# VITA-Group/NeRF-SOS

Hardware: AMD Instinct MI355X
Metric: rays/sec (coarse+fine, 64+128 samples) (higher is better)
Workload: dtype f32; 1 GPU; BASELINE configs[1]: LLFF flower_full shape, 4096 rays/GPU x (64 coarse + 192 fine MLP evaluations), eval-mode NeRFNet.forward, fp32 exact-MFMA, no semantic head, random-init weights (seed 0), pinhole rays 1008x756 f=850; rays_per_gpu=4096, parallelism=ray-sharded x1, no collective in the path

## Files before the change

nerf-sos_amd/csrc/lp_common.h:

```cpp
#pragma once
#include "mlp_common.h"
#include "mlp_host.h"

namespace nsos {
namespace lp {

typedef unsigned u32x4 __attribute__((ext_vector_type(4)));
typedef unsigned u32x2 __attribute__((ext_vector_type(2)));
typedef _Float16 f16x8 __attribute__((ext_vector_type(8)));
typedef __bf16 bf16x8 __attribute__((ext_vector_type(8)));


constexpr int kSlotGroups = 36;
constexpr int kSlotBytes = kSlotGroups * 1024;
constexpr int kSlots = 4;
constexpr int kDmaPieces = kSlotGroups / 4;
constexpr int kTilePts = 256;
#ifdef NSOS_LP_RING
constexpr int kRing = NSOS_LP_RING, kPre = NSOS_LP_RING + 3, kMid = 2;
#else
constexpr int kRing = 5, kPre = 8, kMid = 2;
#endif

constexpr int kAuxAlphaW = 0;
// ... 18 lines not shown
        return __builtin_amdgcn_mfma_f32_32x32x16_f16(__builtin_bit_cast(f16x8, a), __builtin_bit_cast(f16x8, b), c, 0, 0, 0);
    }
    __device__ static __forceinline__ f32x4 mfma_k32(u32x4 a, u32x4 b, f32x4 c) {
        return __builtin_amdgcn_mfma_f32_16x16x32_f16(__builtin_bit_cast(f16x8, a), __builtin_bit_cast(f16x8, b), c, 0, 0, 0);
    }
    __device__ static __forceinline__ unsigned pack2(float lo, float hi) {
        unsigned r;
        asm volatile("v_cvt_pk_f16_f32 %0, %1, %2" : "=v"(r) : "v"(lo), "v"(hi));
        return r;
    }
    __device__ static __forceinline__ float dot2(unsigned a, unsigned b, float acc) {
        asm volatile("v_dot2c_f32_f16 %0, %1, %2" : "+v"(acc) : "v"(a), "v"(b));
        return acc;
    }
    __device__ static __forceinline__ unsigned short bits(float x) {
        const _Float16 h = (_Float16)x;
        return __builtin_bit_cast(unsigned short, h);
    }
};
struct BF16 {
    static constexpr bool kIsF16 = false;
    __device__ static __forceinline__ float lo(unsigned w) { return __builtin_bit_cast(float, w << 16); }
    __device__ static __forceinline__ float hi(unsigned w) { return __builtin_bit_cast(float, w & 0xffff0000u); }
    static constexpr unsigned kOnes = 0x3F803F80u;
    __device__ static __forceinline__ f32x16 mfma(u32x4 a, u32x4 b, f32x16 c) {
        return __builtin_amdgcn_mfma_f32_32x32x16_bf16(__builtin_bit_cast(bf16x8, a), __builtin_bit_cast(bf16x8, b), c, 0, 0, 0);
    }
    __device__ static __forceinline__ f32x4 mfma_k32(u32x4 a, u32x4 b, f32x4 c) {
        return __builtin_amdgcn_mfma_f32_16x16x32_bf16(__builtin_bit_cast(bf16x8, a), __builtin_bit_cast(bf16x8, b), c, 0, 0, 0);
    }
    __device__ static __forceinline__ unsigned pack2(float lo, float hi) {
        unsigned r;
        asm volatile("v_cvt_pk_bf16_f32 %0, %1, %2" : "=v"(r) : "v"(lo), "v"(hi));
        return r;
    }
    __device__ static __forceinline__ float dot2(unsigned a, unsigned b, float acc) {
        asm volatile("v_dot2c_f32_bf16 %0, %1, %2" : "+v"(acc) : "v"(a), "v"(b));
        return acc;
    }
    __device__ static __forceinline__ unsigned short bits(float x) {
        unsigned u = __builtin_bit_cast(unsigned, x);
        if ((u & 0x7fffffffu) > 0x7f800000u) return (unsigned short)((u >> 16) | 0x40);
        u += 0x7fffu + ((u >> 16) & 1u);
        return (unsigned short)(u >> 16);
    }
};

#define NSOS_LP_QUAD(CVT, RELU_OPS)                                                                                  \
    asm volatile("v_accvgpr_read_b32 %0, %8\n\tv_accvgpr_read_b32 %4, %9\n\t"                                        \
                 "v_accvgpr_read_b32 %1, %10\n\tv_accvgpr_read_b32 %5, %11\n\t"                                      \
                 "v_accvgpr_read_b32 %2, %12\n\tv_accvgpr_read_b32 %6, %13\n\t"                                      \
                 "v_accvgpr_read_b32 %3, %14\n\tv_accvgpr_read_b32 %7, %15\n\t" CVT " %0, %0, %4\n\t" CVT          \
                 " %1, %1, %5\n\t" CVT " %2, %2, %6\n\t" CVT " %3, %3, %7" RELU_OPS                                 \
                 : "=&v"(r0), "=&v"(r1), "=&v"(r2), "=&v"(r3), "=&v"(t0), "=&v"(t1), "=&v"(t2), "=&v"(t3)            \
                 : "a"(z[0]), "a"(z[1]), "a"(z[2]), "a"(z[3]), "a"(z[4]), "a"(z[5]), "a"(z[6]), "a"(z[7]))
#define NSOS_LP_RELU4 "\n\tv_pk_max_i16 %0, %0, 0\n\tv_pk_max_i16 %1, %1, 0\n\tv_pk_max_i16 %2, %2, 0\n\tv_pk_max_i16 %3, %3, 0"
template <class T, bool RELU>
__device__ __forceinline__ u32x4 pack8_acc(const float (&z)[8]) {
    unsigned r0, r1, r2, r3, t0, t1, t2, t3;
    if constexpr (T::kIsF16) {
        if constexpr (RELU) NSOS_LP_QUAD("v_cvt_pk_f16_f32", NSOS_LP_RELU4); else NSOS_LP_QUAD("v_cvt_pk_f16_f32", "");
    } else {
        if constexpr (RELU) NSOS_LP_QUAD("v_cvt_pk_bf16_f32", NSOS_LP_RELU4); else NSOS_LP_QUAD("v_cvt_pk_bf16_f32", "");
    }
    return u32x4{r0, r1, r2, r3};
}

struct LpParams {
    const unsigned* aux;
    const unsigned char* chunks;
    const float* rays_o;
    const float* rays_d;
    const float* viewdirs;
    const float* z_vals;
    float* raw;
    long long n_pts;
    int n_samples;
    int n_tiles;
    unsigned long long* prof;
    float* sem_in;
    unsigned* sem_in16;
    float* sem_hid;
    unsigned* sem_hid16;
};
constexpr int kProfSlots = 64;

struct SliceHalf {
    __host__ __device__ static constexpr int of(int idx) { return (idx >> 3) & 1; }
};

template <class T, int L, int S, bool ONE_AT_63>
__device__ __forceinline__ u32x4 enc_slice(const Enc<L, SliceHalf>& e, const float (&x)[3], int kg) {
    u32x4 out;
    static_for<0, 4>([&](auto qc) {
        constexpr int q = decltype(qc)::value, f0 = 16 * S + 2 * q, f1 = 16 * S + 8 + 2 * q;
        const float lo_a = e.template feature<f0, 0>(x), lo_b = e.template feature<f0 + 1, 0>(x);
        const float hi_a = e.template feature<f1, 1>(x);
        const float hi_b = (ONE_AT_63 && f1 + 1 == 63) ? 1.0f : e.template feature<f1 + 1, 1>(x);
        out[q] = T::pack2(kg ? hi_a : lo_a, kg ? hi_b : lo_b);
    });
    return out;
}


template <class T, int NT, bool RELU>
__device__ __forceinline__ void activate(u32x4 (&H)[2][2 * NT], const f32x16 (&Z)[2][NT]) {
    asm volatile("s_nop 15\n\ts_nop 3" ::: "memory");
#pragma unroll
    for (int c = 0; c < 2; ++c)
#pragma unroll
        for (int t = 0; t < NT; ++t)
#pragma unroll
            for (int u = 0; u < 2; ++u) {
                float z[8];
#pragma unroll
                for (int i = 0; i < 8; ++i) z[i] = Z[c][t][8 * u + i];
                H[c][2 * t + u] = pack8_acc<T, RELU>(z);
            }
}

template <int NT, int NO>
__device__ __forceinline__ void heads_partial_f32(const f32x16 (&h)[NT], const float* w_lane, float (&part)[NO]) {
    asm volatile("s_nop 15\n\ts_nop 3" ::: "memory");
#pragma unroll
    for (int t = 0; t < NT; ++t)
#pragma unroll
        for (int q = 0; q < 4; ++q) {
            f32x4 w[NO];
#pragma unroll
            for (int o = 0; o < NO; ++o) w[o] = *reinterpret_cast<const f32x4*>(w_lane + o * 128 + t * 16 + q * 4);
#pragma unroll
            for (int j = 0; j < 4; ++j) {
                float x;
                asm volatile("v_accvgpr_read_b32 %0, %1\n\tv_max_f32 %0, 0, %0" : "=v"(x) : "a"(h[t][q * 4 + j]));
#pragma unroll
                for (int o = 0; o < NO; ++o) part[o] = __fmaf_rn(w[o][j], x, part[o]);
            }
        }
}

template <class F>
int32_t dispatch_lp(int32_t sem_mode, int32_t dtype, bool save, F&& f) {
    return nsos_dispatch_sem(sem_mode, [&](auto sem) -> int32_t {
        return nsos_dispatch_dtype<F16, BF16>(dtype, [&](auto t) -> int32_t {
            return nsos_dispatch_bool(save, [&](auto sv) -> int32_t {
                if constexpr (decltype(sem)::value == 0 && decltype(sv)::value != 0) return NSOS_ERR_UNSUPPORTED;
                else return f(t, sem, sv);
            });
        });
    });
}

__host__ __device__ constexpr int lp16_chunks(int sem) {
    return 1 + 28 + 5 + (sem ? 3 : 1) + 2;
}
constexpr int kLp16TailBytes = 4096;
__host__ __device__ constexpr size_t lp16_stream_bytes(int sem) { return (size_t)lp16_chunks(sem) * kSlotBytes + kLp16TailBytes; }
int32_t launch_lp16(const LpParams& p, int32_t sem_mode, int32_t dtype, bool save, hipStream_t stream);
int32_t pack_lp16(const void* tensors, int32_t sem_mode, bool is_f16, unsigned char* chunks, hipStream_t stream, bool heads_only = false);

}
}
```

nerf-sos_amd/csrc/mlp_lp16.hip:

```cpp
#include "lp_common.h"
#include "lp16_sched.h"

using namespace nsos;
using namespace nsos::lp;

namespace {

constexpr int kRgbLds = kSlots * kSlotBytes + kAuxWords * 4 + kW16 * 768;
template <class T, int NS, int L, int ONE_AT>
__device__ __forceinline__ void encode16(u32x4 (&out)[NS], const float (&x)[3], const unsigned char* lds_tab, int q) {
    constexpr float kInvHi = 0.15915493667125702f, kInvLo = 6.4206382679e-9f;
    float uh[3], ul[3];
#pragma unroll
    for (int c = 0; c < 3; ++c) {
        uh[c] = x[c] * kInvHi;
        ul[c] = __fmaf_rn(x[c], kInvHi, -uh[c]) + x[c] * kInvLo;
    }
    const float amax = fmaxf(fmaxf(fabsf(x[0]), fabsf(x[1])), fabsf(x[2])) * (float)(1 << (L - 1));
    const bool big = !(amax < 32768.0f);
    float val[8 * NS];
    const f32x4* tab = reinterpret_cast<const f32x4*>(lds_tab) + q * (8 * NS);
    static_for<0, 8 * NS>([&](auto jc) {
        constexpr int j = decltype(jc)::value;
        const f32x4 t = tab[j];
        const float ah = __fmaf_rn(uh[2], t[2], __fmaf_rn(uh[1], t[1], uh[0] * t[0]));
        const float fr = __builtin_amdgcn_fractf(ah);
        const float g = __fmaf_rn(ul[0], t[0], __fmaf_rn(ul[1], t[1], __fmaf_rn(ul[2], t[2], fr))) + t[3];
        val[j] = __builtin_amdgcn_sinf(g);
    });
    if (__builtin_expect(big, 0)) {
        static_for<0, 8 * NS>([&](auto jc) {
            constexpr int j = decltype(jc)::value;
            const f32x4 t = tab[j];
            const float a = __fmaf_rn(x[2], t[2], __fmaf_rn(x[1], t[1], x[0] * t[0]));
            float sn, cs;
            sincosf(a, &sn, &cs);
            val[j] = t[3] != 0.0f ? cs : sn;
        });
    }
#pragma unroll
    for (int e = 0; e < 3; ++e) val[e] = q == 0 ? x[e] : val[e];
    constexpr int one_slot = 8 * (NS - 1) + (ONE_AT - 32 * (NS - 1) - 24);
    static_assert(one_slot >= 8 * (NS - 1) && one_slot < 8 * NS, "the constant input lives in lane group 3 of the last slice");
    val[one_slot] = q == 3 ? 1.0f : val[one_slot];
#pragma unroll
    for (int s = 0; s < NS; ++s)
#pragma unroll
        for (int w = 0; w < 4; ++w) out[s][w] = T::pack2(val[8 * s + 2 * w], val[8 * s + 2 * w + 1]);
}

template <class T, int SEM, bool SAVE = false, bool PROF = false>
__global__ __launch_bounds__(64 * kW16, 1) void mlp_lp16_kernel(const LpParams P) {
    extern __shared__ __attribute__((aligned(16))) unsigned char lds[];
    const int lane0 = threadIdx.x & 63, wave = threadIdx.x >> 6;
    constexpr int NCH = lp16_chunks(SEM);
    constexpr int C = SEM ? 6 : 4;

    const unsigned lds_base = (unsigned)(size_t)(__attribute__((address_space(3))) unsigned char*)lds;
    const int wave_s = __builtin_amdgcn_readfirstlane(wave);
    const unsigned voff = (unsigned)(lane0 * 16);
    auto lane_addr = [&](int b) { return lds_base + (unsigned)(b * kSlotBytes + lane0 * 16); };
    auto slot_addr = [&](int b) { return lds_base + (unsigned)(b * kSlotBytes); };
    unsigned c0 = lane_addr(0), c1 = lane_addr(1), c2 = lane_addr(2), c3 = lane_addr(3);
    unsigned d0 = slot_addr(0), d1 = slot_addr(1), d2 = slot_addr(2), d3 = slot_addr(3);
    const unsigned woff = (unsigned)wave_s * 1024u;
    const unsigned wlast = wave_s + kW16 * kFull16 < kSlotGroups ? woff + (unsigned)(kW16 * kFull16) * 1024u : (unsigned)(kSlotGroups - 1) * 1024u;
    auto poff = [&](int i) { return i < kFull16 ? woff + (unsigned)(kW16 * 1024) * (unsigned)i : wlast; };
    const unsigned char* const src_end = P.chunks + (size_t)NCH * kSlotBytes;
    const unsigned char* srcf = P.chunks + (size_t)(2 % NCH) * kSlotBytes;
    auto dma_piece = [&](const unsigned char* src_chunk, unsigned dst_slot, int i) {
        const unsigned long long sp = (unsigned long long)(src_chunk + poff(i));
        const unsigned lo = __builtin_amdgcn_readfirstlane((unsigned)sp), hi = __builtin_amdgcn_readfirstlane((unsigned)(sp >> 32));
        const unsigned dst = __builtin_amdgcn_readfirstlane(dst_slot + poff(i));
        dma_1k(reinterpret_cast<const void*>(((unsigned long long)hi << 32) | lo), dst, voff);
    };
#ifdef NSOS_LP16_DMA_STAGGER
    unsigned fill_wlast = 0;
#endif
    unsigned fill_lo = 0, fill_hi = 0, fill_dst = 0, fill_w = 0;
#ifdef NSOS_LP16_DMA_STAGGER
    auto side = [&](auto early_c, auto late_c) {
        constexpr int EARLY = decltype(early_c)::value, LATE = decltype(late_c)::value;
        auto piece = [&](int i) {
            const unsigned off = i < kFull16 ? fill_w + (unsigned)(kW16 * 1024) * (unsigned)i : fill_wlast;
            const unsigned long long sp = (((unsigned long long)fill_hi << 32) | fill_lo) + off;
            dma_1k(reinterpret_cast<const void*>(sp), fill_dst + off, voff);
        };
        if constexpr (EARLY >= 0 && EARLY < kDma16) { if (wave_s < 4) { NSOS_PIN(); piece(EARLY); NSOS_PIN(); } }
        if constexpr (LATE >= 0 && LATE < kDma16) { if (wave_s >= 4) { NSOS_PIN(); piece(LATE); NSOS_PIN(); } }
    };
#else
    auto side = [&](int i, int nfill) {
        const unsigned off = fill_w + (unsigned)(kW16 * 1024) * (unsigned)i;
        const unsigned long long sp = (((unsigned long long)fill_hi << 32) | fill_lo) + off;
        if (__builtin_constant_p(nfill) && kW16 * i + kW16 - 1 < nfill) {
            dma_1k(reinterpret_cast<const void*>(sp), fill_dst + off, voff);
        } else {
            unsigned keep;
            unsigned long long saved;
            asm volatile("s_mov_b32 %0, m0\n\ts_mov_b32 m0, %2\n\ts_mov_b64 %1, exec\n\ts_cmp_lt_i32 %5, %6\n\ts_cselect_b64 exec, %1, 0\n\ts_nop 2\n\t"
                         "global_load_lds_dwordx4 %3, %4\n\ts_mov_b64 exec, %1\n\ts_mov_b32 m0, %0"
                         : "=&s"(keep), "=&s"(saved) : "s"(fill_dst + off), "v"(voff), "s"(reinterpret_cast<const void*>(sp)), "s"(wave_s + kW16 * i), "s"(nfill)
                         : "memory", "scc");
        }
    };
#endif
    auto mid = [&]() {
        asm volatile("s_waitcnt vmcnt(0)" ::: "memory");
        __builtin_amdgcn_s_barrier();
        const unsigned long long sp = (unsigned long long)srcf;
        fill_lo = __builtin_amdgcn_readfirstlane((unsigned)sp);
        fill_hi = __builtin_amdgcn_readfirstlane((unsigned)(sp >> 32));
        fill_dst = __builtin_amdgcn_readfirstlane(d2);
        fill_w = __builtin_amdgcn_readfirstlane(woff);
#ifdef NSOS_LP16_DMA_STAGGER
        fill_wlast = __builtin_amdgcn_readfirstlane(wlast);
#endif
    };
    auto tail = [&]() {
        const unsigned tc = c0, td = d0;
        c0 = c1; c1 = c2; c2 = c3; c3 = tc;
        d0 = d1; d1 = d2; d2 = d3; d3 = td;
        srcf += kSlotBytes;
        if (srcf == src_end) srcf = P.chunks;
    };
    auto ctx = [&]() { return ChunkCtx{c0, c1}; };

#ifdef NSOS_LP16_PRIO
    if (wave_s >= 4) __builtin_amdgcn_s_setprio(NSOS_LP16_PRIO);
#endif
    f32x4 ring[kRing16];
#pragma unroll
    for (int k = 0; k < 3; ++k)
#pragma unroll
        for (int i = 0; i < kDma16; ++i)
            dma_piece(P.chunks + (size_t)(k % NCH) * kSlotBytes, k == 0 ? d0 : (k == 1 ? d1 : d2), i);
    if (wave_s < 4) {
        const unsigned long long sp = (unsigned long long)(P.chunks + (size_t)NCH * kSlotBytes + (size_t)wave_s * 1024);
        const unsigned lo = __builtin_amdgcn_readfirstlane((unsigned)sp), hi = __builtin_amdgcn_readfirstlane((unsigned)(sp >> 32));
        const unsigned dst = __builtin_amdgcn_readfirstlane(lds_base + (unsigned)(kRgbLds + wave_s * 1024));
        dma_1k(reinterpret_cast<const void*>(((unsigned long long)hi << 32) | lo), dst, voff);
    }
    unsigned char* const tabs = lds + kSlots * kSlotBytes;
    if (threadIdx.x < 64) {
        const int q = threadIdx.x >> 4, j = threadIdx.x & 15;
        reinterpret_cast<f32x4*>(tabs + kTabXyz)[threadIdx.x] = enc_table_entry(32 * (j >> 3) + 8 * q + (j & 7), NSOS_XYZ_FREQS);
    } else if (threadIdx.x < 96) {
        const int i = threadIdx.x - 64, q = i >> 3, j = i & 7;
        reinterpret_cast<f32x4*>(tabs + kTabDir)[i] = enc_table_entry(8 * q + j, NSOS_DIR_FREQS);
    }
    asm volatile("s_waitcnt vmcnt(0)" ::: "memory");
    __syncthreads();
    static_for<0, kRing16>([&](auto ic) { lds_read_a<decltype(ic)::value * 1024>(ring[decltype(ic)::value], c0); });
    NSOS_PIN();

#define IC(n) std::integral_constant<int, (n)> {}
    const f32x4 zero4 = {0.0f, 0.0f, 0.0f, 0.0f};

    if constexpr (PROF)
        if (P.prof && blockIdx.x < 2 && lane0 == 0 && wave_s < 8) P.prof[(blockIdx.x * 8 + wave_s) * kProfSlots + kProfSlots - 2] = __builtin_readcyclecounter();
    for (int tile = blockIdx.x; tile < P.n_tiles; tile += gridDim.x) {
        int lane = lane0;
        asm volatile("" : "+v"(lane));
        const int n = lane & 15, q = lane >> 4;
        int stamp_k = 0;
        auto stamp = [&]() {
            if constexpr (PROF) {
                if (P.prof && tile == (int)(blockIdx.x + gridDim.x) && blockIdx.x < 2) {
                    const unsigned long long t = __builtin_readcyclecounter();
                    if (lane == 0 && stamp_k < kProfSlots && wave_s < 8) P.prof[(blockIdx.x * 8 + wave_s) * kProfSlots + stamp_k] = t;
                }
                ++stamp_k;
            }
        };
        stamp();
        const int n_pts = (int)P.n_pts;
        const int wave_first = tile * kTile16 + wave_s * 32;
        const int n_here = n_pts - wave_first >= 32 ? 32 : (n_pts - wave_first < 0 ? 0 : n_pts - wave_first);
        int* const park = reinterpret_cast<int*>(lds + kSlots * kSlotBytes + kAuxWords * 4) + wave_s * 192 + lane;
        bool save_ok[2] = {false, false};
        unsigned long long save_grp = 0;
        unsigned save_off = 0, save_off_x = 0;
        auto save_store = [&save_grp](auto boff_c, unsigned off, const u32x4& v) {
            constexpr int BOFF = decltype(boff_c)::value;
            unsigned long long b = save_grp + (unsigned long long)(BOFF & ~4095);
            asm volatile("global_store_dwordx4 %0, %1, %2 offset:%3 nt\n\ts_nop 1" : : "v"(off), "v"(v), "s"(b), "i"(BOFF & 4095) : "memory");
        };
        if constexpr (SAVE) {
            save_grp = reinterpret_cast<unsigned long long>(P.sem_in16 + (long long)(wave_first >> 5) * 5120);
            save_off = (unsigned)((2 * (q & 1) + (q >> 1)) * 512 + n * 16);
            save_off_x = (unsigned)(q * 512 + n * 16);
        }
        u32x4 ex[2][2];
        {
#pragma unroll
            for (int c = 0; c < 2; ++c) {
                const int pw = 16 * c + n;
                const bool exists = pw < n_here;
                const int gc = exists ? wave_first + pw : n_pts - 1;
                const int ray = (int)((unsigned)gc / (unsigned)P.n_samples);
                park[64 * c] = ray;
                if constexpr (SAVE) save_ok[c] = exists;
                const float z = P.z_vals[gc];
                float x[3];
#pragma unroll
                for (int k = 0; k < 3; ++k) {
                    const float m = P.rays_d[3ll * ray + k] * z;
                    x[k] = P.rays_o[3ll * ray + k] + m;
                }
                u32x4 e2[2];
#ifdef NSOS_LP16_NOENC
                e2[0] = e2[1] = u32x4{__float_as_uint(x[0]), __float_as_uint(x[1]), __float_as_uint(x[2]), 0u};
#else
                encode16<T, 2, NSOS_XYZ_FREQS, 63>(e2, x, tabs + kTabXyz, q);
#endif
                ex[0][c] = e2[0];
                ex[1][c] = e2[1];
            }
        }

        u32x4 H[8][2];
        f32x4 R[2] = {zero4, zero4};
        auto from_ex = [&](auto sc, auto cc) { return ex[decltype(sc)::value][decltype(cc)::value]; };
        auto store_h7 = [&](auto sc, auto cc) {
            constexpr int s = decltype(sc)::value, c = decltype(cc)::value;
            if constexpr (SAVE) {
                const auto r0 = __builtin_amdgcn_permlane16_swap(H[s][c][0], H[s][c][2], false, false);
                const auto r1 = __builtin_amdgcn_permlane16_swap(H[s][c][1], H[s][c][3], false, false);
#ifndef NSOS_LP16_SKIP_IN
                if (save_ok[c]) save_store(IC(s * 2048 + c * 256), save_off, u32x4{r0[0], r1[0], r0[1], r1[1]});
#endif
            }
        };
        auto store_h7_k = [&](auto kc) { constexpr int k = decltype(kc)::value; store_h7(IC(k >> 1), IC(k & 1)); };
        auto store_ex_k = [&](auto kc) {
            constexpr int k = decltype(kc)::value, s = k >> 1, c = k & 1;
            if constexpr (SAVE)
                if (save_ok[c]) save_store(IC(16 * 1024 + s * 2048 + c * 256), save_off_x, ex[s][c]);
        };

        auto slice_chunk = [&](auto nt_c, auto nsl_c, auto zf_c, auto& acc, auto&& bsel, auto&& ride, const int nfill) {
            constexpr int NT = decltype(nt_c)::value, NSL = decltype(nsl_c)::value;
            constexpr bool ZF = decltype(zf_c)::value != 0;
            pipeline16<NT * NSL, NT * NSL, 0ull>(ring, ctx(), [&](auto ic, const f32x4& a32, const f32x4&) {
                constexpr int g = decltype(ic)::value, sl = g / NT, t = g % NT;
                const u32x4 aop = __builtin_bit_cast(u32x4, a32);
                if constexpr (ZF && sl == 0) {
                    acc[t][0] = T::mfma_k32(aop, bsel(IC(sl), IC(0)), zero4);
                    acc[t][1] = T::mfma_k32(aop, bsel(IC(sl), IC(1)), zero4);
                } else {
                    acc[t][0] = T::mfma_k32(aop, bsel(IC(sl), IC(0)), acc[t][0]);
                    acc[t][1] = T::mfma_k32(aop, bsel(IC(sl), IC(1)), acc[t][1]);
                }
                ride(ic);
            }, mid, tail, side, nfill);
#pragma unroll
            for (int t = 0; t < NT; ++t) asm volatile("" : "+v"(acc[t][0]), "+v"(acc[t][1]));
        };
        auto quad_chunk = [&](auto extra_c, auto& zq, auto&& ride, auto&& extra, const int nfill) {
            constexpr unsigned long long EXTRA = (unsigned long long)decltype(extra_c)::value;
            pipeline16x<32, 32, 0ull, EXTRA>(ring, ctx(), [&](auto ic, const f32x4& a32, const f32x4&) {
                constexpr int g = decltype(ic)::value, s = g >> 2, t = g & 3;
                const u32x4 aop = __builtin_bit_cast(u32x4, a32);
                if constexpr (s == 0) {
                    zq[t][1] = T::mfma_k32(aop, H[0][1], zq[t][0]);
                    zq[t][0] = T::mfma_k32(aop, H[0][0], zq[t][0]);
                } else {
                    zq[t][0] = T::mfma_k32(aop, H[s][0], zq[t][0]);
                    zq[t][1] = T::mfma_k32(aop, H[s][1], zq[t][1]);
                }
#ifndef NSOS_LP16_NORIDE
                ride(ic);
#endif
            }, mid, tail, side, extra, nfill);
#pragma unroll
            for (int t = 0; t < 4; ++t) asm volatile("" : "+v"(zq[t][0]), "+v"(zq[t][1]));
        };
        auto read_bias = [&](auto tc, f32x4& dst, unsigned slot_lane) {
            constexpr int t = decltype(tc)::value;
            const unsigned addr = slot_lane - (unsigned)(lane * 16) + (unsigned)(q * 16);
            asm volatile("ds_read_b128 %0, %1 offset:%2" : "=v"(dst) : "v"(addr), "i"(32768 + 64 * t) : "memory");
        };
        auto no_ride = [](auto) {};
        auto quad_word = [&](auto& zq, int ls, int c, int w) {
            return T::pack2(zq[2 * ls + (w >> 1)][c][2 * (w & 1)], zq[2 * ls + (w >> 1)][c][2 * (w & 1) + 1]);
        };

        stamp();
        f32x4 Zq[2][4][2];
        auto dead = [&]() {
#pragma unroll
            for (int b = 0; b < 2; ++b)
#pragma unroll
                for (int t = 0; t < 4; ++t) asm volatile("" : "=v"(Zq[b][t][0]), "=v"(Zq[b][t][1]));
        };
        auto activate_all = [&](const f32x4 (&Z)[16][2]) {
            asm volatile("s_nop 7" ::: "memory");
#pragma unroll
            for (int s = 0; s < 8; ++s) {
#pragma unroll
                for (int c = 0; c < 2; ++c)
#pragma unroll
                    for (int w = 0; w < 4; ++w) H[s][c][w] = T::pack2(Z[2 * s + (w >> 1)][c][2 * (w & 1)], Z[2 * s + (w >> 1)][c][2 * (w & 1) + 1]);
#pragma unroll
                for (int c = 0; c < 2; ++c)
#pragma unroll
                    for (int w = 0; w < 4; ++w) NSOS_RELU_WORD16(H[s][c][w], 0u);
            }
        };
        {
            f32x4 Z[16][2];
            slice_chunk(IC(16), IC(2), IC(1), Z, from_ex, [&](auto gc_) {
                constexpr int g = decltype(gc_)::value;
                if constexpr (SAVE && SEM != 0 && g >= 3 && g < 15 && g % 3 == 0) store_ex_k(IC(g / 3 - 1));
            }, 33);
            stamp();
            activate_all(Z);
            stamp();
        }
        auto quad_layer = [&](const int l, const bool tail_pending, const bool leave_tail, const bool bias_now, const bool next_quad) {
            const unsigned floor = l < 8 ? 0u : 0x80008000u;
            u32x4 Ho[4][2];
            if (bias_now) {
                static_for<0, 4>([&](auto tc) { read_bias(tc, Zq[0][decltype(tc)::value][0], c0); });
                lgkm_wait<0>();
                asm volatile("" : "+v"(Zq[0][0][0]), "+v"(Zq[0][1][0]), "+v"(Zq[0][2][0]), "+v"(Zq[0][3][0]));
            }
            auto ride_tail = [&](auto gc_) {
                constexpr int g = decltype(gc_)::value;
                if constexpr (g >= 4 && g <= 20) {
                    if (tail_pending) {
                        if constexpr (g >= 5) {
                            constexpr int k = g - 5;
                            NSOS_RELU_WORD16(H[6 + (k >> 3)][(k >> 2) & 1][k & 3], 0u);
                        }
                        if constexpr (g < 20) {
                            constexpr int k = g - 4;
                            H[6 + (k >> 3)][(k >> 2) & 1][k & 3] = quad_word(Zq[1], k >> 3, (k >> 2) & 1, k & 3);
                        }
                    }
                }
            };
            auto ride_act = [&](auto gc_, auto src_c, auto base_c) {
                constexpr int g = decltype(gc_)::value, SRC = decltype(src_c)::value, BASE = decltype(base_c)::value;
                if constexpr (g >= 5 && g <= 20) {
                    constexpr int k = g - 5;
                    NSOS_RELU_WORD16(Ho[BASE + (k >> 3)][(k >> 2) & 1][k & 3], floor);
                }
                if constexpr (g >= 4 && g < 20) {
                    constexpr int k = g - 4;
                    Ho[BASE + (k >> 3)][(k >> 2) & 1][k & 3] = quad_word(Zq[SRC], k >> 3, (k >> 2) & 1, k & 3);
                }
            };
            auto ride_save = [&](auto gc_, auto ch_c) {
                constexpr int g = decltype(gc_)::value, CH = decltype(ch_c)::value;
                if constexpr (SAVE && SEM != 0 && g >= 3 && (g - 3) % 6 == 0 && (g - 3) / 6 < (CH == 2 ? 2 : 3))
                    if (l == 8) store_h7_k(IC(8 + 3 * CH + (g - 3) / 6));
            };
            constexpr unsigned long long kBiasAt = 0xFull << 24;
            quad_chunk(std::integral_constant<unsigned long long, kBiasAt>{}, Zq[0], [&](auto gc_) { ride_tail(gc_); ride_save(gc_, IC(0)); },
                       [&](auto gc_) { read_bias(IC(decltype(gc_)::value - 24), Zq[1][decltype(gc_)::value - 24][0], c1); }, 33);
            quad_chunk(std::integral_constant<unsigned long long, kBiasAt>{}, Zq[1], [&](auto gc_) { ride_act(gc_, IC(0), IC(0)); ride_save(gc_, IC(1)); },
                       [&](auto gc_) { read_bias(IC(decltype(gc_)::value - 24), Zq[0][decltype(gc_)::value - 24][0], c1); }, 33);
            const int nfill_next = l == 8 ? 36 : 33;
            quad_chunk(std::integral_constant<unsigned long long, kBiasAt>{}, Zq[0], [&](auto gc_) { ride_act(gc_, IC(1), IC(2)); ride_save(gc_, IC(2)); },
                       [&](auto gc_) { read_bias(IC(decltype(gc_)::value - 24), Zq[1][decltype(gc_)::value - 24][0], c1); }, nfill_next);
            quad_chunk(std::integral_constant<unsigned long long, 0ull>{}, Zq[1], [&](auto gc_) {
                constexpr int g = decltype(gc_)::value;
                if constexpr (g >= 4 && g <= 17 && ((g - 4) & 3) < 2) mov_slice16(H[(g - 4) >> 2][(g - 4) & 1], Ho[(g - 4) >> 2][(g - 4) & 1]);
                if constexpr (g >= 21 && g <= 28) { constexpr int k = g - 21; NSOS_RELU_WORD16(H[4][k >> 2][k & 3], floor); }
                if constexpr (g >= 25) { constexpr int k = g - 25; NSOS_RELU_WORD16(H[5][k >> 2][k & 3], floor); }
                if constexpr (g >= 20 && g <= 27) { constexpr int k = g - 20; H[4][k >> 2][k & 3] = quad_word(Zq[0], 0, k >> 2, k & 3); }
                if constexpr (g >= 24) { constexpr int k = g - 24; H[5][k >> 2][k & 3] = quad_word(Zq[0], 1, k >> 2, k & 3); }
                if constexpr (g == 22 || g == 24 || g == 26 || g == 28) {
                    if (next_quad) { NSOS_PIN(); read_bias(IC((g - 22) >> 1), Zq[0][(g - 22) >> 1][0], c1); NSOS_PIN(); }
                }
            }, [](auto) {}, nfill_next);
            NSOS_RELU_WORD16(H[5][1][3], floor);
            stamp();
            if (!leave_tail) {
                asm volatile("s_nop 7" ::: "memory");
#pragma unroll
                for (int k = 0; k < 16; ++k) H[6 + (k >> 3)][(k >> 2) & 1][k & 3] = quad_word(Zq[1], k >> 3, (k >> 2) & 1, k & 3);
#pragma unroll
                for (int k = 0; k < 16; ++k) NSOS_RELU_WORD16(H[6 + (k >> 3)][(k >> 2) & 1][k & 3], floor);
            }
            stamp();
        };
        dead();
#pragma unroll 1
        for (int l = 1; l <= 4; ++l) quad_layer(l, l != 1, l != 4, l == 1, l != 4);
        dead();
        {
            f32x4 Z[16][2];
            auto from_H01 = [&](auto sc, auto cc) { return H[0 + decltype(sc)::value][decltype(cc)::value]; };
            auto from_H23 = [&](auto sc, auto cc) { return H[2 + decltype(sc)::value][decltype(cc)::value]; };
            auto from_H45 = [&](auto sc, auto cc) { return H[4 + decltype(sc)::value][decltype(cc)::value]; };
            auto from_H67 = [&](auto sc, auto cc) { return H[6 + decltype(sc)::value][decltype(cc)::value]; };
            slice_chunk(IC(16), IC(2), IC(1), Z, from_H01, no_ride, 32);
            slice_chunk(IC(16), IC(2), IC(0), Z, from_H23, no_ride, 32);
            slice_chunk(IC(16), IC(2), IC(0), Z, from_H45, no_ride, 32);
            slice_chunk(IC(16), IC(2), IC(0), Z, from_H67, no_ride, 33);
            slice_chunk(IC(16), IC(2), IC(0), Z, from_ex, no_ride, 33);
            stamp();
            activate_all(Z);
            stamp();
        }
        dead();
#pragma unroll 1
        for (int l = 6; l <= 8; ++l) {
            quad_layer(l, l == 7, l == 6, l != 7, l == 6);
            if (l == 7) {
                dead();
                if constexpr (SEM == 0) {
                    pipeline16<12, 9, 0x1ull>(ring, ctx(), [&](auto ic, const f32x4& a32, const f32x4& prev) {
                        constexpr int g = decltype(ic)::value;
                        const u32x4 aop = __builtin_bit_cast(u32x4, a32);
                        if constexpr (g == 1) {
                            R[0] = T::mfma_k32(aop, H[0][0], prev);
                            R[1] = T::mfma_k32(aop, H[0][1], prev);
                        } else if constexpr (g >= 2 && g < 9) {
                            R[0] = T::mfma_k32(aop, H[g - 1][0], R[0]);
                            R[1] = T::mfma_k32(aop, H[g - 1][1], R[1]);
                        }
                    }, mid, tail, side, 33);
                    asm volatile("" : "+v"(R[0]), "+v"(R[1]));
                } else {
                    f32x4 S8[8][2];
                    u32x4 Sp[4][2];
                    auto from_Hlo = [&](auto sc, auto cc) { return H[decltype(sc)::value][decltype(cc)::value]; };
                    auto from_Hhi = [&](auto sc, auto cc) { return H[4 + decltype(sc)::value][decltype(cc)::value]; };
                    auto ride_sem = [&](auto gc_, auto ch_c) {
                        constexpr int g = decltype(gc_)::value, CH = decltype(ch_c)::value;
                        if constexpr (SAVE && g >= 3 && (g - 3) % 6 == 0 && (g - 3) / 6 < (CH == 2 ? 2 : 3)) store_h7_k(IC(3 * CH + (g - 3) / 6));
                    };
                    slice_chunk(IC(8), IC(4), IC(1), S8, from_Hlo, [&](auto gc_) { ride_sem(gc_, IC(0)); }, SEM == 2 ? 29 : 21);
#ifdef NSOS_LP16_HEAD_STAMPS
                    stamp();
#endif
                    slice_chunk(IC(8), IC(4), IC(0), S8, from_Hhi, [&](auto gc_) { ride_sem(gc_, IC(1)); }, 33);
#ifdef NSOS_LP16_HEAD_STAMPS
                    stamp();
#endif
                    auto activate_sem = [&]() {
                        asm volatile("s_nop 7" ::: "memory");
#pragma unroll
                        for (int s = 0; s < 4; ++s)
#pragma unroll
                            for (int c = 0; c < 2; ++c)
#pragma unroll
                                for (int w = 0; w < 4; ++w) Sp[s][c][w] = T::pack2(S8[2 * s + (w >> 1)][c][2 * (w & 1)], S8[2 * s + (w >> 1)][c][2 * (w & 1) + 1]);
#pragma unroll
                        for (int s = 0; s < 4; ++s)
#pragma unroll
                            for (int c = 0; c < 2; ++c)
#pragma unroll
                                for (int w = 0; w < 4; ++w) NSOS_RELU_WORD16(Sp[s][c][w], 0u);
                        if constexpr (SAVE) {
                            const unsigned long long hid_grp = reinterpret_cast<unsigned long long>(P.sem_hid16 + (long long)(wave_first >> 5) * 2048);
#pragma unroll
                            for (int s = 0; s < 4; ++s)
#pragma unroll
                                for (int c = 0; c < 2; ++c) {
                                    const auto r0 = __builtin_amdgcn_permlane16_swap(Sp[s][c][0], Sp[s][c][2], false, false);
                                    const auto r1 = __builtin_amdgcn_permlane16_swap(Sp[s][c][1], Sp[s][c][3], false, false);
                                    const u32x4 v = {r0[0], r1[0], r0[1], r1[1]};
#ifndef NSOS_LP16_SKIP_HID
                                    if (save_ok[c])
                                        asm volatile("global_store_dwordx4 %0, %1, %2 offset:%3 nt\n\ts_nop 1" : : "v"(save_off), "v"(v), "s"(hid_grp + (unsigned long long)((s * 2048 + c * 256) & ~4095)),
                                                     "i"((s * 2048 + c * 256) & 4095) : "memory");
#endif
                                }
                        }
                    };
                    if constexpr (SEM == 2) {
                        pipeline16<32, 29, 1ull << 16>(ring, ctx(), [&](auto ic, const f32x4& a32, const f32x4& prev) {
                            constexpr int g = decltype(ic)::value;
                            const u32x4 aop = __builtin_bit_cast(u32x4, a32);
                            if constexpr (g < 16) {
                                constexpr int sl = g >> 3, t = g & 7;
                                S8[t][0] = T::mfma_k32(aop, ex[sl][0], S8[t][0]);
                                S8[t][1] = T::mfma_k32(aop, ex[sl][1], S8[t][1]);
                            } else if constexpr (g == 17) {
                                R[0] = T::mfma_k32(aop, H[0][0], prev);
                                R[1] = T::mfma_k32(aop, H[0][1], prev);
                            } else if constexpr (g >= 18 && g < 25) {
                                R[0] = T::mfma_k32(aop, H[g - 17][0], R[0]);
                                R[1] = T::mfma_k32(aop, H[g - 17][1], R[1]);
                            } else if constexpr (g >= 25 && g < 29) {
                                if constexpr (g == 25) activate_sem();
                                R[0] = T::mfma_k32(aop, Sp[g - 25][0], R[0]);
                                R[1] = T::mfma_k32(aop, Sp[g - 25][1], R[1]);
                            }
                            ride_sem(ic, IC(2));
                        }, mid, tail, side, 33);
                    } else {
                        const unsigned one_w = q == 0 ? (unsigned)(T::kOnes & 0xffffu) : 0u;
                        const u32x4 ones = {one_w, 0u, 0u, 0u};
                        pipeline16<24, 21, 1ull << 8>(ring, ctx(), [&](auto ic, const f32x4& a32, const f32x4& prev) {
                            constexpr int g = decltype(ic)::value;
                            const u32x4 aop = __builtin_bit_cast(u32x4, a32);
                            if constexpr (g < 8) {
                                S8[g][0] = T::mfma_k32(aop, ones, S8[g][0]);
                                S8[g][1] = T::mfma_k32(aop, ones, S8[g][1]);
                            } else if constexpr (g == 9) {
                                R[0] = T::mfma_k32(aop, H[0][0], prev);
                                R[1] = T::mfma_k32(aop, H[0][1], prev);
                            } else if constexpr (g >= 10 && g < 17) {
                                R[0] = T::mfma_k32(aop, H[g - 9][0], R[0]);
                                R[1] = T::mfma_k32(aop, H[g - 9][1], R[1]);
                            } else if constexpr (g >= 17 && g < 21) {
                                if constexpr (g == 17) activate_sem();
                                R[0] = T::mfma_k32(aop, Sp[g - 17][0], R[0]);
                                R[1] = T::mfma_k32(aop, Sp[g - 17][1], R[1]);
                            }
                            ride_sem(ic, IC(2));
                        }, mid, tail, side, 33);
                    }
                    asm volatile("" : "+v"(R[0]), "+v"(R[1]));
                }
                stamp();
            }
        }
        dead();
        u32x4 ed[2];
        {
#pragma unroll
            for (int c = 0; c < 2; ++c) {
                const int ray_c = park[64 * c];
                float dv[3];
#pragma unroll
                for (int k = 0; k < 3; ++k) dv[k] = P.viewdirs[3ll * ray_c + k];
                u32x4 e1[1];
                encode16<T, 1, NSOS_DIR_FREQS, 27>(e1, dv, tabs + kTabDir, q);
                ed[c] = e1[0];
            }
        }
        stamp();
        u32x4 Vp[4][2];
        auto view_chunk = [&](auto& zq, auto&& ride, const int nfill) {
            pipeline16<36, 36, 0ull>(ring, ctx(), [&](auto ic, const f32x4& a32, const f32x4&) {
                constexpr int g = decltype(ic)::value, s = g >> 2, t = g & 3;
                const u32x4 aop = __builtin_bit_cast(u32x4, a32);
                if constexpr (s == 0) {
                    zq[t][0] = T::mfma_k32(aop, H[0][0], zero4);
                    zq[t][1] = T::mfma_k32(aop, H[0][1], zero4);
                } else if constexpr (s < 8) {
                    zq[t][0] = T::mfma_k32(aop, H[s][0], zq[t][0]);
                    zq[t][1] = T::mfma_k32(aop, H[s][1], zq[t][1]);
                } else {
                    zq[t][0] = T::mfma_k32(aop, ed[0], zq[t][0]);
                    zq[t][1] = T::mfma_k32(aop, ed[1], zq[t][1]);
                }
                ride(ic);
            }, mid, tail, side, nfill);
#pragma unroll
            for (int t = 0; t < 4; ++t) asm volatile("" : "+v"(zq[t][0]), "+v"(zq[t][1]));
        };
        view_chunk(Zq[0], no_ride, 32);
        view_chunk(Zq[1], [&](auto gc_) {
            constexpr int g = decltype(gc_)::value;
            if constexpr (g >= 9 && g <= 24) { constexpr int k = g - 9; NSOS_RELU_WORD16(Vp[k >> 3][(k >> 2) & 1][k & 3], 0u); }
            if constexpr (g >= 8 && g < 24) { constexpr int k = g - 8; Vp[k >> 3][(k >> 2) & 1][k & 3] = quad_word(Zq[0], k >> 3, (k >> 2) & 1, k & 3); }
        }, 33);
        stamp();
        {
            asm volatile("s_nop 7" ::: "memory");
#pragma unroll
            for (int k = 0; k < 16; ++k) Vp[2 + (k >> 3)][(k >> 2) & 1][k & 3] = quad_word(Zq[1], k >> 3, (k >> 2) & 1, k & 3);
#pragma unroll
            for (int k = 0; k < 16; ++k) NSOS_RELU_WORD16(Vp[2 + (k >> 3)][(k >> 2) & 1][k & 3], 0u);
        }
        float chk[2];
#pragma unroll
        for (int c = 0; c < 2; ++c) {
            const int ray_c = park[64 * c];
            int pw = 16 * c + n;
            asm volatile("" : "+v"(pw));
            const int gc_b = (pw < n_here) ? wave_first + pw : n_pts - 1;
            const float nz = P.z_vals[gc_b];
            float acc = nz - nz;
#pragma unroll
            for (int k = 0; k < 3; ++k) {
                const float o = P.rays_o[3ll * ray_c + k], d = P.rays_d[3ll * ray_c + k], v = P.viewdirs[3ll * ray_c + k];
                acc += ((o - o) + (d - d)) + (v - v);
            }
            chk[c] = acc;
        }
        {
            f32x4 ra[4];
            const unsigned ra_addr = lds_base + (unsigned)kRgbLds + (unsigned)(lane * 16);
            static_for<0, 4>([&](auto kc) { lds_read_a<decltype(kc)::value * 1024>(ra[decltype(kc)::value], ra_addr); });
            asm volatile("s_waitcnt lgkmcnt(0)" : "+v"(ra[0]), "+v"(ra[1]), "+v"(ra[2]), "+v"(ra[3]) : : "memory");
#pragma unroll
            for (int k = 0; k < 4; ++k) {
                const u32x4 aop = __builtin_bit_cast(u32x4, ra[k]);
                R[0] = T::mfma_k32(aop, Vp[k][0], R[0]);
                R[1] = T::mfma_k32(aop, Vp[k][1], R[1]);
            }
        }
        asm volatile("" : "+v"(R[0]), "+v"(R[1]));
        stamp();
        {
            asm volatile("s_nop 7" ::: "memory");
#pragma unroll
            for (int c = 0; c < 2; ++c)
                if (chk[c] != chk[c]) {
                    const float qnan = __builtin_nanf("");
                    R[c] = f32x4{qnan, qnan, qnan, qnan};
                }
            if constexpr (C == 4) {
#pragma unroll
                for (int c = 0; c < 2; ++c)
                    if (q == 0 && 16 * c + n < n_here) *reinterpret_cast<f32x4*>(P.raw + (long long)(wave_first + 16 * c + n) * 4) = R[c];
            } else {
                float* const stage = reinterpret_cast<float*>(lds + kSlots * kSlotBytes + kAuxWords * 4) + wave_s * 192;
                __builtin_amdgcn_fence(__ATOMIC_RELEASE, "wavefront");
                __builtin_amdgcn_wave_barrier();
                if (n_here == 32) {
#pragma unroll
                    for (int c = 0; c < 2; ++c) {
                        if (q == 0) {
                            *reinterpret_cast<f32x2*>(stage + 6 * (16 * c + n)) = f32x2{R[c][0], R[c][1]};
                            *reinterpret_cast<f32x2*>(stage + 6 * (16 * c + n) + 2) = f32x2{R[c][2], R[c][3]};
                        }
                        if (q == 1) *reinterpret_cast<f32x2*>(stage + 6 * (16 * c + n) + 4) = f32x2{R[c][0], R[c][1]};
                    }
                    __builtin_amdgcn_fence(__ATOMIC_RELEASE, "wavefront");
                    __builtin_amdgcn_wave_barrier();
                    __builtin_amdgcn_fence(__ATOMIC_ACQUIRE, "wavefront");
                    if (lane < 48) *reinterpret_cast<f32x4*>(P.raw + (long long)wave_first * C + 4 * lane) = *reinterpret_cast<const f32x4*>(stage + 4 * lane);
                    __builtin_amdgcn_fence(__ATOMIC_RELEASE, "wavefront");
                    __builtin_amdgcn_wave_barrier();
                } else {
#pragma unroll
                    for (int c = 0; c < 2; ++c)
                        if (16 * c + n < n_here) {
                            float* out = P.raw + (long long)(wave_first + 16 * c + n) * C;
                            if (q == 0) {
                                *reinterpret_cast<f32x2*>(out) = f32x2{R[c][0], R[c][1]};
                                *reinterpret_cast<f32x2*>(out + 2) = f32x2{R[c][2], R[c][3]};
                            } else if (q == 1) {
                                *reinterpret_cast<f32x2*>(out + 4) = f32x2{R[c][0], R[c][1]};
                            }
                        }
                }
            }
        }
        stamp();
    }
#undef IC
    if constexpr (PROF)
        if (P.prof && blockIdx.x < 2 && lane0 == 0 && wave_s < 8) P.prof[(blockIdx.x * 8 + wave_s) * kProfSlots + kProfSlots - 1] = __builtin_readcyclecounter();
    asm volatile("s_waitcnt vmcnt(0) lgkmcnt(0)" ::: "memory");
    __syncthreads();
}

constexpr int kLdsBytes16 = kRgbLds + kLp16TailBytes;
static_assert(kLdsBytes16 <= 160 * 1024, "LDS");

template <class T, int SEM, bool SAVE, bool PROF>
int32_t launch16p(const LpParams& p, hipStream_t stream) {
    LpParams q = p;
    q.n_tiles = (int)((p.n_pts + kTile16 - 1) / kTile16);
    return nsos_launch_persistent<&mlp_lp16_kernel<T, SEM, SAVE, PROF>>(q, q.n_tiles, 64 * kW16, kLdsBytes16, stream);
}
template <class T, int SEM, bool SAVE>
int32_t launch16(const LpParams& p, hipStream_t stream) {
    if (p.prof) {
        if constexpr (SEM != 1) return launch16p<T, SEM, SAVE, true>(p, stream);
        else return NSOS_ERR_UNSUPPORTED;
    }
    return launch16p<T, SEM, SAVE, false>(p, stream);
}

enum Kind16 { kQ16 = 0,
              kSlice16 = 1,
              kEnc16 = 2,
              kView16 = 3,
              kSemTail2 = 4, kSemTail1 = 5, kSigma16 = 6, kRgb16 = 7 };
struct Chunk16 {
    const float* w;
    const float* bias;
    int in_dim, col_base, kind, a0, nt;
};
struct Pack16Params {
    Chunk16 ch[48];
    int n_chunks;
    int first, count;
    int tail;
    const float* alpha_w; const float* alpha_b;
    const float* rgb_w; const float* rgb_b;
    const float* sem0_w; const float* sem0_b;
    const float* sem2_w; const float* sem2_b;
    unsigned short* chunks;
};

__device__ __forceinline__ int hid_col(int s, int q, int e) { return 32 * s + 16 * (e >> 2) + 4 * q + (e & 3); }

template <class T>
__global__ __launch_bounds__(256) void lp16_pack_kernel(const Pack16Params P) {
    const long long gid = (long long)blockIdx.x * blockDim.x + threadIdx.x;
    const long long per_chunk = kSlotBytes / 2;
    const long long body = (long long)P.count * per_chunk;
    if (gid >= body + (P.tail ? kLp16TailBytes / 2 : 0)) return;
    const bool in_tail = gid >= body;
    const Chunk16 ck = in_tail ? Chunk16{nullptr, nullptr, 0, 0, kRgb16, 0, 0} : P.ch[P.first + gid / per_chunk];
    const int within = in_tail ? (int)(gid - body) : (int)(gid % per_chunk);
    const int g = within >> 9, lane = (within >> 3) & 63, e = within & 7;
    const int i = lane & 15, q = lane >> 4;
    const int W = NSOS_NET_WIDTH, X = NSOS_XYZ_DIM;
    bool is_bias = false;
    float v = 0.0f;
    auto raw_bias = [&]() {
        is_bias = true;
        const int row = 4 * q + (e >> 1);
        v = row < 3 ? P.rgb_b[row] : row == 3 ? P.alpha_b[0] : (row < 6 && P.sem2_b) ? P.sem2_b[row - 4] : 0.0f;
    };
    auto sigma_a = [&](int s) { v = i == 3 ? P.alpha_w[hid_col(s, q, e)] : 0.0f; };
    auto logits_a = [&](int s) { v = (i == 4 || i == 5) ? P.sem2_w[(i - 4) * (W / 2) + hid_col(s, q, e)] : 0.0f; };
    switch (ck.kind) {
        case kQ16: {
            if (g < 32) {
                const int sl = g >> 2, t = 4 * ck.a0 + (g & 3);
                v = ck.w[(long long)(16 * t + i) * ck.in_dim + ck.col_base + hid_col(sl, q, e)];
            } else if (g == 32) {
                const int word = (lane * 8 + e) >> 1;
                if (word < 64) {
                    is_bias = true;
                    v = ck.bias ? ck.bias[16 * (4 * ck.a0 + (word >> 4)) + (word & 15)] : 0.0f;
                }
            }
        } break;
        case kSlice16: {
            if (g < 32) {
                const int s = ck.a0 + g / ck.nt, t = g % ck.nt;
                v = ck.w[(long long)(16 * t + i) * ck.in_dim + ck.col_base + hid_col(s, q, e)];
            }
        } break;
        case kEnc16: {
            if (g < 2 * ck.nt) {
                const int s = g / ck.nt, t = g % ck.nt, f = 32 * s + 8 * q + e;
                if (f < X) v = ck.w[(long long)(16 * t + i) * ck.in_dim + ck.col_base + f];
                else if (f == 63 && ck.bias) v = ck.bias[16 * t + i];
            }
        } break;
        case kView16: {
            const int s = g >> 2, t = 4 * ck.a0 + (g & 3);
            if (s < 8) v = ck.w[(long long)(16 * t + i) * ck.in_dim + hid_col(s, q, e)];
            else {
                const int f = 8 * q + e;
                if (f < NSOS_DIR_DIM) v = ck.w[(long long)(16 * t + i) * ck.in_dim + W + f];
                else if (f == 27) v = ck.bias[16 * t + i];
            }
        } break;
        case kSemTail2: {
            if (g < 16) {
                const int s = g >> 3, t = g & 7, f = 32 * s + 8 * q + e;
                if (f < X) v = P.sem0_w[(long long)(16 * t + i) * (W + X) + W + f];
                else if (f == 63) v = P.sem0_b[16 * t + i];
            } else if (g == 16) raw_bias();
            else if (g < 25) sigma_a(g - 17);
            else if (g < 29) logits_a(g - 25);
        } break;
        case kSemTail1: {
            if (g < 8) v = (q == 0 && e == 0) ? P.sem0_b[16 * g + i] : 0.0f;
            else if (g == 8) raw_bias();
            else if (g < 17) sigma_a(g - 9);
            else if (g < 21) logits_a(g - 17);
        } break;
        case kSigma16: {
            if (g == 0) raw_bias();
            else if (g < 9) sigma_a(g - 1);
        } break;
        case kRgb16: {
            if (g < 4) v = i < 3 ? P.rgb_w[i * (W / 2) + hid_col(g, q, e)] : 0.0f;
        } break;
    }
    const long long at = in_tail ? (long long)P.n_chunks * per_chunk + within : (long long)P.first * per_chunk + gid;
    if (is_bias) {
        const unsigned u = __builtin_bit_cast(unsigned, v);
        P.chunks[at] = (e & 1) ? (unsigned short)(u >> 16) : (unsigned short)(u & 0xffffu);
    } else {
        P.chunks[at] = T::bits(v);
    }
}

}

namespace nsos {
namespace lp {

int32_t pack_lp16(const void* tensors, int32_t sem_mode, bool is_f16, unsigned char* chunks, hipStream_t stream, bool heads_only) {
    const nsos_mlp_tensors* T_ = static_cast<const nsos_mlp_tensors*>(tensors);
    const int X = NSOS_XYZ_DIM, W = NSOS_NET_WIDTH;
    Pack16Params P = {};
    int n = 0;
    auto add = [&](const float* w, const float* bias, int in_dim, int col, int kind, int a0, int nt) {
        P.ch[n++] = Chunk16{w, bias, in_dim, col, kind, a0, nt};
    };
    auto quads = [&](const float* w, const float* b) {
        for (int c = 0; c < 4; ++c) add(w, b, W, 0, kQ16, c, 4);
    };
    add(T_->pts_w[0], T_->pts_b[0], X, 0, kEnc16, 0, 16);
    for (int l = 1; l <= 4; ++l) quads(T_->pts_w[l], T_->pts_b[l]);
    for (int j = 0; j < 4; ++j) add(T_->pts_w[5], nullptr, X + W, X, kSlice16, 2 * j, 16);
    add(T_->pts_w[5], T_->pts_b[5], X + W, 0, kEnc16, 0, 16);
    quads(T_->pts_w[6], T_->pts_b[6]);
    quads(T_->pts_w[7], T_->pts_b[7]);
    if (sem_mode) {
        const int in_dim = sem_mode == NSOS_SEM_COORD ? W + X : W;
        for (int j = 0; j < 2; ++j) add(T_->sem0_w, nullptr, in_dim, 0, kSlice16, 4 * j, 8);
        add(nullptr, nullptr, 0, 0, sem_mode == NSOS_SEM_COORD ? kSemTail2 : kSemTail1, 0, 0);
    } else {
        add(nullptr, nullptr, 0, 0, kSigma16, 0, 0);
    }
    quads(T_->feature_w, T_->feature_b);
    for (int j = 0; j < 2; ++j) add(T_->views_w, T_->views_b, W + NSOS_DIR_DIM, 0, kView16, j, 4);
    if (n != lp16_chunks(sem_mode)) return NSOS_ERR_UNSUPPORTED;
    P.n_chunks = n;
    P.first = heads_only ? 30 : 0;
    P.count = heads_only ? 3 : n;
    P.alpha_w = T_->alpha_w; P.alpha_b = T_->alpha_b;
    P.rgb_w = T_->rgb_w; P.rgb_b = T_->rgb_b;
    P.sem0_w = sem_mode ? T_->sem0_w : nullptr; P.sem0_b = sem_mode ? T_->sem0_b : nullptr;
    P.sem2_w = sem_mode ? T_->sem2_w : nullptr; P.sem2_b = sem_mode ? T_->sem2_b : nullptr;
    P.chunks = reinterpret_cast<unsigned short*>(chunks);
    P.tail = heads_only ? 0 : 1;
    const long long total = (long long)P.count * (kSlotBytes / 2) + (P.tail ? kLp16TailBytes / 2 : 0);
    const dim3 grid((unsigned)((total + 255) / 256)), block(256);
    if (is_f16) hipLaunchKernelGGL(lp16_pack_kernel<F16>, grid, block, 0, stream, P);
    else hipLaunchKernelGGL(lp16_pack_kernel<BF16>, grid, block, 0, stream, P);
    return nsos_launch_status();
}

int32_t launch_lp16(const LpParams& p, int32_t sem_mode, int32_t dtype, bool save, hipStream_t st) {
    return dispatch_lp(sem_mode, dtype, save, [&](auto t, auto sem, auto sv) -> int32_t {
        return launch16<decltype(t), decltype(sem)::value, decltype(sv)::value != 0>(p, st);
    });
}

}
}
```

Baseline: 538,300 rays/s.

## Fold feature linear layer into views layer weights to drop a hidden layer

Removes the separate feature_linear quad layer (no activation between feature and views layers) by precomputing views_w·feature_w and the folded bias in double precision at weight-pack time. This removes one 256x256 MFMA layer per point from the kernel, so the per-tile weight stream shrinks from 28 to 24 quad chunks. The layer loop now ends at 7, the h7 save path moves into the view chunks, and pad chunks keep the stream size unchanged. The risk is an extra rounding difference from the folded low-precision weights, plus the schedule and fill-count changes.

```diff
diff --git a/nerf-sos_amd/csrc/lp_common.h b/nerf-sos_amd/csrc/lp_common.h
--- a/nerf-sos_amd/csrc/lp_common.h
+++ b/nerf-sos_amd/csrc/lp_common.h
@@ -194,8 +194,9 @@
 }
 
 __host__ __device__ constexpr int lp16_chunks(int sem) {
-    return 1 + 28 + 5 + (sem ? 3 : 1) + 2;
-}
+    return 1 + 24 + 5 + (sem ? 3 : 1) + 2 + 4;
+}
+constexpr int kLp16PadChunks = 4;
 constexpr int kLp16TailBytes = 4096;
 __host__ __device__ constexpr size_t lp16_stream_bytes(int sem) { return (size_t)lp16_chunks(sem) * kSlotBytes + kLp16TailBytes; }
 int32_t launch_lp16(const LpParams& p, int32_t sem_mode, int32_t dtype, bool save, hipStream_t stream);
diff --git a/nerf-sos_amd/csrc/mlp_lp16.hip b/nerf-sos_amd/csrc/mlp_lp16.hip
--- a/nerf-sos_amd/csrc/mlp_lp16.hip
+++ b/nerf-sos_amd/csrc/mlp_lp16.hip
@@ -53,7 +53,7 @@
 __global__ __launch_bounds__(64 * kW16, 1) void mlp_lp16_kernel(const LpParams P) {
     extern __shared__ __attribute__((aligned(16))) unsigned char lds[];
     const int lane0 = threadIdx.x & 63, wave = threadIdx.x >> 6;
-    constexpr int NCH = lp16_chunks(SEM);
+    constexpr int NCH = lp16_chunks(SEM) - kLp16PadChunks;
     constexpr int C = SEM ? 6 : 4;
 
     const unsigned lds_base = (unsigned)(size_t)(__attribute__((address_space(3))) unsigned char*)lds;
@@ -136,7 +136,7 @@
         for (int i = 0; i < kDma16; ++i)
             dma_piece(P.chunks + (size_t)(k % NCH) * kSlotBytes, k == 0 ? d0 : (k == 1 ? d1 : d2), i);
     if (wave_s < 4) {
-        const unsigned long long sp = (unsigned long long)(P.chunks + (size_t)NCH * kSlotBytes + (size_t)wave_s * 1024);
+        const unsigned long long sp = (unsigned long long)(P.chunks + (size_t)lp16_chunks(SEM) * kSlotBytes + (size_t)wave_s * 1024);
         const unsigned lo = __builtin_amdgcn_readfirstlane((unsigned)sp), hi = __builtin_amdgcn_readfirstlane((unsigned)(sp >> 32));
         const unsigned dst = __builtin_amdgcn_readfirstlane(lds_base + (unsigned)(kRgbLds + wave_s * 1024));
         dma_1k(reinterpret_cast<const void*>(((unsigned long long)hi << 32) | lo), dst, voff);
@@ -319,7 +319,7 @@
             stamp();
         }
         auto quad_layer = [&](const int l, const bool tail_pending, const bool leave_tail, const bool bias_now, const bool next_quad) {
-            const unsigned floor = l < 8 ? 0u : 0x80008000u;
+            constexpr unsigned floor = 0u;
             u32x4 Ho[4][2];
             if (bias_now) {
                 static_for<0, 4>([&](auto tc) { read_bias(tc, Zq[0][decltype(tc)::value][0], c0); });
@@ -352,19 +352,14 @@
                     Ho[BASE + (k >> 3)][(k >> 2) & 1][k & 3] = quad_word(Zq[SRC], k >> 3, (k >> 2) & 1, k & 3);
                 }
             };
-            auto ride_save = [&](auto gc_, auto ch_c) {
-                constexpr int g = decltype(gc_)::value, CH = decltype(ch_c)::value;
-                if constexpr (SAVE && SEM != 0 && g >= 3 && (g - 3) % 6 == 0 && (g - 3) / 6 < (CH == 2 ? 2 : 3))
-                    if (l == 8) store_h7_k(IC(8 + 3 * CH + (g - 3) / 6));
-            };
             constexpr unsigned long long kBiasAt = 0xFull << 24;
-            quad_chunk(std::integral_constant<unsigned long long, kBiasAt>{}, Zq[0], [&](auto gc_) { ride_tail(gc_); ride_save(gc_, IC(0)); },
+            quad_chunk(std::integral_constant<unsigned long long, kBiasAt>{}, Zq[0], ride_tail,
                        [&](auto gc_) { read_bias(IC(decltype(gc_)::value - 24), Zq[1][decltype(gc_)::value - 24][0], c1); }, 33);
-            quad_chunk(std::integral_constant<unsigned long long, kBiasAt>{}, Zq[1], [&](auto gc_) { ride_act(gc_, IC(0), IC(0)); ride_save(gc_, IC(1)); },
+            quad_chunk(std::integral_constant<unsigned long long, kBiasAt>{}, Zq[1], [&](auto gc_) { ride_act(gc_, IC(0), IC(0)); },
                        [&](auto gc_) { read_bias(IC(decltype(gc_)::value - 24), Zq[0][decltype(gc_)::value - 24][0], c1); }, 33);
-            const int nfill_next = l == 8 ? 36 : 33;
-            quad_chunk(std::integral_constant<unsigned long long, kBiasAt>{}, Zq[0], [&](auto gc_) { ride_act(gc_, IC(1), IC(2)); ride_save(gc_, IC(2)); },
-                       [&](auto gc_) { read_bias(IC(decltype(gc_)::value - 24), Zq[1][decltype(gc_)::value - 24][0], c1); }, nfill_next);
+            const int nfill_last = (SEM == 0 && l == 7) ? 36 : 33;
+            quad_chunk(std::integral_constant<unsigned long long, kBiasAt>{}, Zq[0], [&](auto gc_) { ride_act(gc_, IC(1), IC(2)); },
+                       [&](auto gc_) { read_bias(IC(decltype(gc_)::value - 24), Zq[1][decltype(gc_)::value - 24][0], c1); }, 33);
             quad_chunk(std::integral_constant<unsigned long long, 0ull>{}, Zq[1], [&](auto gc_) {
                 constexpr int g = decltype(gc_)::value;
                 if constexpr (g >= 4 && g <= 17 && ((g - 4) & 3) < 2) mov_slice16(H[(g - 4) >> 2][(g - 4) & 1], Ho[(g - 4) >> 2][(g - 4) & 1]);
@@ -375,7 +370,7 @@
                 if constexpr (g == 22 || g == 24 || g == 26 || g == 28) {
                     if (next_quad) { NSOS_PIN(); read_bias(IC((g - 22) >> 1), Zq[0][(g - 22) >> 1][0], c1); NSOS_PIN(); }
                 }
-            }, [](auto) {}, nfill_next);
+            }, [](auto) {}, nfill_last);
             NSOS_RELU_WORD16(H[5][1][3], floor);
             stamp();
             if (!leave_tail) {
@@ -408,8 +403,8 @@
         }
         dead();
 #pragma unroll 1
-        for (int l = 6; l <= 8; ++l) {
-            quad_layer(l, l == 7, l == 6, l != 7, l == 6);
+        for (int l = 6; l <= 7; ++l) {
+            quad_layer(l, l == 7, l == 6, l == 6, l == 6);
             if (l == 7) {
                 dead();
                 if constexpr (SEM == 0) {
@@ -423,7 +418,7 @@
                             R[0] = T::mfma_k32(aop, H[g - 1][0], R[0]);
                             R[1] = T::mfma_k32(aop, H[g - 1][1], R[1]);
                         }
-                    }, mid, tail, side, 33);
+                    }, mid, tail, side, 36);
                     asm volatile("" : "+v"(R[0]), "+v"(R[1]));
                 } else {
                     f32x4 S8[8][2];
@@ -438,7 +433,7 @@
 #ifdef NSOS_LP16_HEAD_STAMPS
                     stamp();
 #endif
-                    slice_chunk(IC(8), IC(4), IC(0), S8, from_Hhi, [&](auto gc_) { ride_sem(gc_, IC(1)); }, 33);
+                    slice_chunk(IC(8), IC(4), IC(0), S8, from_Hhi, [&](auto gc_) { ride_sem(gc_, IC(1)); }, 36);
 #ifdef NSOS_LP16_HEAD_STAMPS
                     stamp();
 #endif
@@ -493,7 +488,7 @@
                                 R[1] = T::mfma_k32(aop, Sp[g - 25][1], R[1]);
                             }
                             ride_sem(ic, IC(2));
-                        }, mid, tail, side, 33);
+                        }, mid, tail, side, 36);
                     } else {
                         const unsigned one_w = q == 0 ? (unsigned)(T::kOnes & 0xffffu) : 0u;
                         const u32x4 ones = {one_w, 0u, 0u, 0u};
@@ -515,7 +510,7 @@
                                 R[1] = T::mfma_k32(aop, Sp[g - 17][1], R[1]);
                             }
                             ride_sem(ic, IC(2));
-                        }, mid, tail, side, 33);
+                        }, mid, tail, side, 36);
                     }
                     asm volatile("" : "+v"(R[0]), "+v"(R[1]));
                 }
@@ -557,9 +552,14 @@
 #pragma unroll
             for (int t = 0; t < 4; ++t) asm volatile("" : "+v"(zq[t][0]), "+v"(zq[t][1]));
         };
-        view_chunk(Zq[0], no_ride, 32);
+        auto ride_view = [&](auto gc_, auto ch_c) {
+            constexpr int g = decltype(gc_)::value, CH = decltype(ch_c)::value;
+            if constexpr (SAVE && g >= 3 && (g - 3) % 6 == 0 && (g - 3) / 6 < 4) store_h7_k(IC(8 + 4 * CH + (g - 3) / 6));
+        };
+        view_chunk(Zq[0], [&](auto gc_) { ride_view(gc_, IC(0)); }, 32);
         view_chunk(Zq[1], [&](auto gc_) {
             constexpr int g = decltype(gc_)::value;
+            ride_view(gc_, IC(1));
             if constexpr (g >= 9 && g <= 24) { constexpr int k = g - 9; NSOS_RELU_WORD16(Vp[k >> 3][(k >> 2) & 1][k & 3], 0u); }
             if constexpr (g >= 8 && g < 24) { constexpr int k = g - 8; Vp[k >> 3][(k >> 2) & 1][k & 3] = quad_word(Zq[0], k >> 3, (k >> 2) & 1, k & 3); }
         }, 33);
@@ -678,7 +678,8 @@
               kSlice16 = 1,
               kEnc16 = 2,
               kView16 = 3,
-              kSemTail2 = 4, kSemTail1 = 5, kSigma16 = 6, kRgb16 = 7 };
+              kSemTail2 = 4, kSemTail1 = 5, kSigma16 = 6, kRgb16 = 7,
+              kPad16 = 8 };
 struct Chunk16 {
     const float* w;
     const float* bias;
@@ -693,10 +694,18 @@
     const float* rgb_w; const float* rgb_b;
     const float* sem0_w; const float* sem0_b;
     const float* sem2_w; const float* sem2_b;
+    const float* feat_w; const float* feat_b;
     unsigned short* chunks;
 };
 
 __device__ __forceinline__ int hid_col(int s, int q, int e) { return 32 * s + 16 * (e >> 2) + 4 * q + (e & 3); }
+
+__device__ __forceinline__ double fold_dot(const float* a, const float* b, int ldb) {
+    double acc = 0.0;
+#pragma unroll 8
+    for (int j = 0; j < NSOS_NET_WIDTH; ++j) acc = __dadd_rn(acc, __dmul_rn((double)a[j], (double)b[(long long)j * ldb]));
+    return acc;
+}
 
 template <class T>
 __global__ __launch_bounds__(256) void lp16_pack_kernel(const Pack16Params P) {
@@ -747,13 +756,15 @@
         } break;
         case kView16: {
             const int s = g >> 2, t = 4 * ck.a0 + (g & 3);
-            if (s < 8) v = ck.w[(long long)(16 * t + i) * ck.in_dim + hid_col(s, q, e)];
+            const float* wv = ck.w + (long long)(16 * t + i) * ck.in_dim;
+            if (s < 8) v = (float)fold_dot(wv, P.feat_w + hid_col(s, q, e), W);
             else {
                 const int f = 8 * q + e;
-                if (f < NSOS_DIR_DIM) v = ck.w[(long long)(16 * t + i) * ck.in_dim + W + f];
-                else if (f == 27) v = ck.bias[16 * t + i];
+                if (f < NSOS_DIR_DIM) v = wv[W + f];
+                else if (f == 27) v = (float)__dadd_rn(fold_dot(wv, P.feat_b, 1), (double)ck.bias[16 * t + i]);
             }
         } break;
+        case kPad16: break;
         case kSemTail2: {
             if (g < 16) {
                 const int s = g >> 3, t = g & 7, f = 32 * s + 8 * q + e;
@@ -815,8 +826,8 @@
     } else {
         add(nullptr, nullptr, 0, 0, kSigma16, 0, 0);
     }
-    quads(T_->feature_w, T_->feature_b);
     for (int j = 0; j < 2; ++j) add(T_->views_w, T_->views_b, W + NSOS_DIR_DIM, 0, kView16, j, 4);
+    for (int j = 0; j < kLp16PadChunks; ++j) add(nullptr, nullptr, 0, 0, kPad16, 0, 0);
     if (n != lp16_chunks(sem_mode)) return NSOS_ERR_UNSUPPORTED;
     P.n_chunks = n;
     P.first = heads_only ? 30 : 0;
@@ -825,6 +836,7 @@
     P.rgb_w = T_->rgb_w; P.rgb_b = T_->rgb_b;
     P.sem0_w = sem_mode ? T_->sem0_w : nullptr; P.sem0_b = sem_mode ? T_->sem0_b : nullptr;
     P.sem2_w = sem_mode ? T_->sem2_w : nullptr; P.sem2_b = sem_mode ? T_->sem2_b : nullptr;
+    P.feat_w = T_->feature_w; P.feat_b = T_->feature_b;
     P.chunks = reinterpret_cast<unsigned short*>(chunks);
     P.tail = heads_only ? 0 : 1;
     const long long total = (long long)P.count * (kSlotBytes / 2) + (P.tail ? kLp16TailBytes / 2 : 0);
```

New measurement: 538,200 rays/s. About the same (-0.0%).
